# YuhuaXu/ImageMosaicing

Measured on AMD Instinct MI355X. Metric: image-pairs/sec (detect+match+H+warp), 4000x3000 UAV frames, higher is better.
Workload: dtype i16 fixed-point pyramid filtered in f32 (as the reference's OpenCV), f32 (RANSAC / warp coordinates), int8 MFMA with int32 accumulation (descriptor distances, exact), u8 (pixels); 1 GPU; C3: ONE 500-frame 4000x3000 UAV survey, pair window 2 (499 pairs), SIFT(2000,3,0.01,20) + exact BF match + 3x3 grid select + Ransac2D + MosaicImagesRefined warp; frames=500, pairs=499, frames_per_gpu=500, pairs_per_gpu=499

## Files before the change

imagemosaicing_amd/csrc/sift.hip:

```cpp
#include "common.h"
#include <memory>
#include "detmath.h"
#include <cmath>
#include <type_traits>

namespace {

constexpr int N_LAYERS = 3, N_LEVELS = 6, IMG_BORDER = 5, MAX_INTERP = 5, ORI_BINS = 36, MAX_OCT = 16;
constexpr int FIXPT_SCALE = 48;
constexpr float DOG_THRESHOLD_P1 = 21.0f;
constexpr float HIST_Q = 1024.0f;
constexpr int MAX_R = 16;
constexpr int SIFT_BATCH_MAX = MI355_SIFT_BATCH_MAX;
typedef int16_t lvl_t;

__host__ __device__ __forceinline__ int reflect101(int p, int n) {
    if (n == 1) return 0;
    while (p < 0 || p >= n) { if (p < 0) p = -p; else p = 2 * n - 2 - p; }
    return p;
}

typedef float v2f __attribute__((ext_vector_type(2)));
struct __attribute__((aligned(4))) uint2_a4 { unsigned x, y; };
typedef float v4f __attribute__((ext_vector_type(4)));
// ... 321 lines not shown
        }
    }
    __syncthreads();
    for (int item = tid; item < EH * (EW / 4); item += 256) {
        const int ly = item / (EW / 4), xg = item - ly * (EW / 4);
        const int r = y0 + ly;
        float cm[5][6], cn[5][6], mid[5][6], top[5][6], bot[5][6];
#pragma unroll
        for (int pl = 0; pl < 5; pl++) {
            const float* base = reinterpret_cast<const float*>(s_d4[pl]) + (ly + 1) * PC + 4 * xg + 4;
#pragma unroll
            for (int rr = -1; rr <= 1; rr++) {
                const float* q = base + rr * PC;
                const v4f c4 = *reinterpret_cast<const v4f*>(q);
                float v[6] = {q[-1], c4.x, c4.y, c4.z, c4.w, q[4]};
#pragma unroll
                for (int j = 0; j < 6; j++) { if (rr == -1) top[pl][j] = v[j]; else if (rr == 0) mid[pl][j] = v[j]; else bot[pl][j] = v[j]; }
            }
#pragma unroll
            for (int j = 0; j < 6; j++) {
                cm[pl][j] = fmaxf(fmaxf(top[pl][j], mid[pl][j]), bot[pl][j]);
                cn[pl][j] = fminf(fminf(top[pl][j], mid[pl][j]), bot[pl][j]);
            }
        }
        unsigned hit = 0;
#pragma unroll
        for (int k = 0; k < 4; k++) {
            const int j = k + 1;
#pragma unroll
            for (int layer = 1; layer <= N_LAYERS; layer++) {
                const float val = mid[layer][j];
                float mx = fmaxf(fmaxf(cm[layer - 1][j - 1], cm[layer - 1][j]), cm[layer - 1][j + 1]);
                mx = fmaxf(mx, fmaxf(fmaxf(cm[layer + 1][j - 1], cm[layer + 1][j]), cm[layer + 1][j + 1]));
                mx = fmaxf(mx, fmaxf(fmaxf(cm[layer][j - 1], cm[layer][j + 1]), fmaxf(top[layer][j], bot[layer][j])));
                float mn = fminf(fminf(cn[layer - 1][j - 1], cn[layer - 1][j]), cn[layer - 1][j + 1]);
                mn = fminf(mn, fminf(fminf(cn[layer + 1][j - 1], cn[layer + 1][j]), cn[layer + 1][j + 1]));
                mn = fminf(mn, fminf(fminf(cn[layer][j - 1], cn[layer][j + 1]), fminf(top[layer][j], bot[layer][j])));
                const float q = val > 0.0f ? mx : -mn;
                hit |= fabsf(val) >= fmaxf(q, DOG_THRESHOLD_P1) ? (1u << ((layer - 1) * 4 + k)) : 0u;
            }
        }
        unsigned cmask = 0;
#pragma unroll
        for (int k = 0; k < 4; k++) { const int c = x0 + 4 * xg + k; cmask |= (c >= IMG_BORDER && c < oc.w - IMG_BORDER) ? (0x111u << k) : 0u; }
        hit = (r >= IMG_BORDER && r < oc.h - IMG_BORDER) ? (hit & cmask) : 0u;
        while (hit) {
            const int bb = __builtin_ctz(hit); hit &= hit - 1;
            const int layer = bb / 4 + 1, c = x0 + 4 * xg + (bb & 3);
            const unsigned long long rec = ((unsigned long long)octave << 48) | ((unsigned long long)layer << 40) | ((unsigned long long)r << 20) | (unsigned long long)c;
            const unsigned slot = atomicAdd(&s_n, 1u);
            if (slot < ECAP) s_list[slot] = rec;
            else {
                const unsigned reg = ((unsigned)tile >> REG_SHIFT) & (NREG - 1);
                const unsigned g = atomicAdd(&count[reg * REG_STRIDE], 1u);
                if (g < cap) cand[(size_t)reg * cap + g] = rec; else *overflow = 1;
            }
        }
    }
    __syncthreads();
    const unsigned nloc = s_n < ECAP ? s_n : ECAP;
    const unsigned reg = ((unsigned)tile >> REG_SHIFT) & (NREG - 1);
    if (tid == 0 && nloc) s_base = atomicAdd(&count[reg * REG_STRIDE], nloc);
    __syncthreads();
    for (unsigned i = tid; i < nloc; i += 256) {
        const unsigned g = s_base + i;
        if (g < cap) cand[(size_t)reg * cap + g] = s_list[i] | (g < cube_cap ? (1ull << 63) : 0ull); else *overflow = 1;
    }
    for (unsigned idx = tid; idx < nloc * 27; idx += 256) {
        const unsigned ci = idx / 27, e = idx - ci * 27;
        const unsigned g = s_base + ci;
        if (g >= cube_cap) continue;
        const unsigned long long rec = s_list[ci];
        const int L0 = (int)((rec >> 40) & 0xff), R0 = (int)((rec >> 20) & 0xfffff), C0 = (int)(rec & 0xfffff);
        const int dl = (int)(e / 9) - 1, dr = (int)((e / 3) % 3) - 1, dc = (int)(e % 3) - 1;
        cube[((size_t)reg * 32 + e) * cube_cap + g] = reinterpret_cast<const float*>(s_d4[L0 + dl])[(R0 + dr - y0 + 1) * PC + (C0 + dc - x0) + 4];
    }
}

constexpr int XCAP = 512;
#ifndef MI355_XD
#define MI355_XD 2
#endif
constexpr int XD = MI355_XD;
#ifndef MI355_XWAVES
#define MI355_XWAVES 3
#endif
constexpr int XWAVES = MI355_XWAVES;
constexpr int XSW = 248;
typedef short s2 __attribute__((ext_vector_type(2)));
struct XRow { uint2 m[N_LEVELS]; };
struct XDog { s2 m[5][2]; };
__device__ __forceinline__ s2 as_s2(unsigned v) { return __builtin_bit_cast(s2, v); }
__device__ __forceinline__ unsigned as_u(s2 v) { return __builtin_bit_cast(unsigned, v); }
__device__ __forceinline__ s2 pmax(s2 a, s2 b) { return __builtin_elementwise_max(a, b); }
__device__ __forceinline__ s2 pmin(s2 a, s2 b) { return __builtin_elementwise_min(a, b); }
__device__ __forceinline__ unsigned dpp_lower(unsigned v) { return (unsigned)__builtin_amdgcn_update_dpp(0, (int)v, 0x138 , 0xf, 0xf, true); }
__device__ __forceinline__ unsigned dpp_upper(unsigned v) { return (unsigned)__builtin_amdgcn_update_dpp(0, (int)v, 0x130 , 0xf, 0xf, true); }

__device__ __forceinline__ unsigned xtest_row(const XDog& A, const XDog& B, const XDog& C, int xm, int clo, int chi, bool row_ok) {
    s2 hx[5][2], hn[5][2];
#pragma unroll
    for (int p = 0; p < 5; p++) {
        auto h3 = [](s2 c01, s2 c23, bool mx, s2& o01, s2& o23) {
            const unsigned u01 = as_u(c01), u23 = as_u(c23);
            const unsigned l23 = dpp_lower(u23), r01 = dpp_upper(u01);
            const s2 s_m0 = as_s2(__builtin_amdgcn_alignbit(u01, l23, 16));
            const s2 s_12 = as_s2(__builtin_amdgcn_alignbit(u23, u01, 16));
            const s2 s_34 = as_s2(__builtin_amdgcn_alignbit(r01, u23, 16));
            if (mx) { o01 = pmax(pmax(s_m0, c01), s_12); o23 = pmax(pmax(s_12, c23), s_34); }
            else    { o01 = pmin(pmin(s_m0, c01), s_12); o23 = pmin(pmin(s_12, c23), s_34); }
        };
        h3(pmax(pmax(A.m[p][0], B.m[p][0]), C.m[p][0]), pmax(pmax(A.m[p][1], B.m[p][1]), C.m[p][1]), true, hx[p][0], hx[p][1]);
        h3(pmin(pmin(A.m[p][0], B.m[p][0]), C.m[p][0]), pmin(pmin(A.m[p][1], B.m[p][1]), C.m[p][1]), false, hn[p][0], hn[p][1]);
    }
    unsigned hit = 0;
    const s2 t21 = {21, 21}, tm21 = {-21, -21};
#pragma unroll
    for (int layer = 1; layer <= N_LAYERS; layer++) {
#pragma unroll
        for (int r = 0; r < 2; r++) {
            const s2 val = B.m[layer][r];
            const s2 mx = pmax(pmax(pmax(hx[layer - 1][r], hx[layer][r]), hx[layer + 1][r]), t21);
            const s2 mn = pmin(pmin(pmin(hn[layer - 1][r], hn[layer][r]), hn[layer + 1][r]), tm21);
            const bool h0 = (val.x == mx.x) | (val.x == mn.x), h1 = (val.y == mx.y) | (val.y == mn.y);
            hit = (hit << 2) | (h0 ? 2u : 0u) | (h1 ? 1u : 0u);
        }
    }
    if (!row_ok || hit == 0) return 0u;
    unsigned out = 0;
#pragma unroll
    for (int b = 0; b < 12; b++) out |= ((hit >> (11 - b)) & 1u) << b;
    unsigned cmask = 0;
#pragma unroll
    for (int k = 0; k < 4; k++) cmask |= (xm + k >= clo && xm + k < chi) ? (0x111u << k) : 0u;
    return out & cmask;
}

struct XH { s2 hx[5][2], hn[5][2]; };
struct XCen { s2 v[3][2]; };
__device__ __forceinline__ void xrow_extremes(const XDog& d, XH& h, XCen& c) {
#pragma unroll
    for (int p = 0; p < 5; p++) {
        const unsigned u01 = as_u(d.m[p][0]), u23 = as_u(d.m[p][1]);
        const unsigned l23 = dpp_lower(u23), r01 = dpp_upper(u01);
        const s2 s_m0 = as_s2(__builtin_amdgcn_alignbit(u01, l23, 16));
        const s2 s_12 = as_s2(__builtin_amdgcn_alignbit(u23, u01, 16));
        const s2 s_34 = as_s2(__builtin_amdgcn_alignbit(r01, u23, 16));
        h.hx[p][0] = pmax(pmax(s_m0, d.m[p][0]), s_12); h.hx[p][1] = pmax(pmax(s_12, d.m[p][1]), s_34);
        h.hn[p][0] = pmin(pmin(s_m0, d.m[p][0]), s_12); h.hn[p][1] = pmin(pmin(s_12, d.m[p][1]), s_34);
    }
#pragma unroll
    for (int l = 0; l < 3; l++) { c.v[l][0] = d.m[l + 1][0]; c.v[l][1] = d.m[l + 1][1]; }
}
__device__ __forceinline__ unsigned xtest_rows(const XH& A, const XH& B, const XH& C, const XCen& cen, int xm, int clo, int chi, bool row_ok) {
    s2 hx[5][2], hn[5][2];
#pragma unroll
    for (int p = 0; p < 5; p++)
#pragma unroll
        for (int r = 0; r < 2; r++) { hx[p][r] = pmax(pmax(A.hx[p][r], B.hx[p][r]), C.hx[p][r]); hn[p][r] = pmin(pmin(A.hn[p][r], B.hn[p][r]), C.hn[p][r]); }
    unsigned hit = 0;
    const s2 t21 = {21, 21}, tm21 = {-21, -21};
#pragma unroll
    for (int layer = 1; layer <= N_LAYERS; layer++) {
#pragma unroll
        for (int r = 0; r < 2; r++) {
            const s2 val = cen.v[layer - 1][r];
            const s2 mx = pmax(pmax(pmax(hx[layer - 1][r], hx[layer][r]), hx[layer + 1][r]), t21);
            const s2 mn = pmin(pmin(pmin(hn[layer - 1][r], hn[layer][r]), hn[layer + 1][r]), tm21);
            const bool h0 = (val.x == mx.x) | (val.x == mn.x), h1 = (val.y == mx.y) | (val.y == mn.y);
            hit = (hit << 2) | (h0 ? 2u : 0u) | (h1 ? 1u : 0u);
        }
    }
    if (!row_ok || hit == 0) return 0u;
    unsigned out = 0;
#pragma unroll
    for (int b = 0; b < 12; b++) out |= ((hit >> (11 - b)) & 1u) << b;
    unsigned cmask = 0;
#pragma unroll
    for (int k = 0; k < 4; k++) cmask |= (xm + k >= clo && xm + k < chi) ? (0x111u << k) : 0u;
    return out & cmask;
}

__global__ __launch_bounds__(256) __attribute__((amdgpu_waves_per_eu(XWAVES, XWAVES)))
void extrema_stream(OctaveDev oc, int octave, unsigned long long* cand, unsigned* count, unsigned cap, unsigned* overflow, BatchStride bs,
                    float* cube, unsigned cube_cap, int L, int nstrip, int nseg, int nb, int xsw ) {
    const int lane = threadIdx.x & 63, wave = threadIdx.x >> 6;
    int unit = __builtin_amdgcn_readfirstlane(xcd_remap(blockIdx.x, gridDim.x) * 4 + wave);
    const int per = nstrip * nseg, fr = unit / per;
    if (fr >= nb) return;
    unit -= fr * per;
    {
        const size_t f = (size_t)fr;
#pragma unroll
        for (int l = 0; l < N_LEVELS; l++) oc.lv[l] += f * bs.pyr;
        cand += f * bs.cand; count += f * CCNT_STRIDE; overflow += f * CNT_STRIDE; cube += f * bs.cube;
    }
    const int seg = unit / nstrip, strip = unit - seg * nstrip;
    const int xs = strip * xsw, y0 = seg * L;
    const int lact = (oc.h - y0 < L) ? oc.h - y0 : L;
    const unsigned reg = (unsigned)unit & (NREG - 1);
    const int xm = xs - 4 + 4 * lane;
    const int xl = xm < 0 ? 0 : (xm < oc.w - 4 ? xm : oc.w - 4);
    int clo = xs > IMG_BORDER ? xs : IMG_BORDER, chi = xs + xsw < oc.w - IMG_BORDER ? xs + xsw : oc.w - IMG_BORDER;
    if (lane == 0 || lane == 63) { clo = 0; chi = 0; }
    const int hm1 = oc.h - 1;
    auto load_row = [&](int r, XRow& q) {
        r = r < 0 ? 0 : (r > hm1 ? hm1 : r);
        const size_t o = (size_t)r * oc.w + xl;
#pragma unroll
        for (int l = 0; l < N_LEVELS; l++) q.m[l] = *reinterpret_cast<const uint2*>(oc.lv[l] + o);
    };
    auto to_dog = [&](const XRow& q, XDog& d) {
#pragma unroll
        for (int p = 0; p < 5; p++) { d.m[p][0] = as_s2(q.m[p + 1].x) - as_s2(q.m[p].x); d.m[p][1] = as_s2(q.m[p + 1].y) - as_s2(q.m[p].y); }
    };
    __shared__ unsigned long long s_rec[4][XCAP];
    int nq = 0;
    auto wave_sync = [&]() { __builtin_amdgcn_fence(__ATOMIC_ACQ_REL, "wavefront"); __builtin_amdgcn_wave_barrier(); };
    auto flush = [&]() {
        if (nq == 0) return;
        wave_sync();
        unsigned base = 0;
        if (lane == 0) base = atomicAdd(&count[reg * REG_STRIDE], (unsigned)nq);
        base = __shfl(base, 0);
        for (int idx = lane; idx < nq; idx += 64) {
            const unsigned g = base + (unsigned)idx;
            if (g >= cap) { *overflow = 1; continue; }
            cand[(size_t)reg * cap + g] = s_rec[wave][idx];
        }
        wave_sync();
        nq = 0;
    };
    auto emit = [&](unsigned hit, int rc, auto in_loop) -> bool {
        constexpr bool IN_LOOP = decltype(in_loop)::value;
        const int nq0 = nq;
        while (__builtin_amdgcn_ballot_w64(hit != 0)) {
            const bool mine = hit != 0;
            const int bb = mine ? __builtin_ctz(hit) : 0;
            hit &= hit - 1;
            const unsigned long long m = __builtin_amdgcn_ballot_w64(mine);
            const int add = __builtin_popcountll(m);
            if (nq + add > XCAP) {
                if constexpr (IN_LOOP) { nq = nq0; return false; }
                else flush();
            }
            if (mine) {
                const int layer = bb / 4 + 1, c = xm + (bb & 3);
                s_rec[wave][nq + __builtin_popcountll(m & ((1ull << lane) - 1ull))] =
                    ((unsigned long long)octave << 48) | ((unsigned long long)layer << 40) | ((unsigned long long)rc << 20) | (unsigned long long)c;
            }
            nq += add;
        }
        return true;
    };
    XH win[3];
    XCen cen[3];
    XRow nxt[XD];
    {
        XRow q; XDog dq;
        load_row(y0 - 1, q); to_dog(q, dq); xrow_extremes(dq, win[0], cen[0]);
        load_row(y0, q); to_dog(q, dq); xrow_extremes(dq, win[1], cen[1]);
#pragma unroll
        for (int d = 0; d < XD; d++) load_row(y0 + 1 + d, nxt[d]);
    }
    int tb = 0, t_slow = -1;
    for (bool done = false; !done;) {
        for (;;) {
            if (tb >= lact) { done = true; break; }
            if (nq > XCAP / 2) break;
            auto step = [&](auto jc) -> bool {
                constexpr int j = decltype(jc)::value;
                const int tt = tb + j;
                if (tt >= lact) return false;
                const int rc = y0 + tt;
                XH& A = win[j % 3]; XH& B = win[(j + 1) % 3]; XH& Cc = win[(j + 2) % 3];
                { XDog dq; to_dog(nxt[j % XD], dq); xrow_extremes(dq, Cc, cen[(j + 2) % 3]); }
                load_row(rc + 1 + XD, nxt[j % XD]);
                const unsigned hit = xtest_rows(A, B, Cc, cen[(j + 1) % 3], xm, clo, chi, rc >= IMG_BORDER && rc < oc.h - IMG_BORDER);
                if (!emit(hit, rc, std::true_type{})) { t_slow = tt; return false; }
                return true;
            };
            if (!static_rows<0, 3 * XD>(step)) { done = true; break; }
            tb += 3 * XD;
        }
        flush();
    }
    if (t_slow >= 0) {
        for (int tt = t_slow; tt < lact; tt++) {
            const int rc = y0 + tt;
            XRow q; XDog A, B, Cc;
            load_row(rc - 1, q); to_dog(q, A);
            load_row(rc, q); to_dog(q, B);
            load_row(rc + 1, q); to_dog(q, Cc);
            emit(xtest_row(A, B, Cc, xm, clo, chi, rc >= IMG_BORDER && rc < oc.h - IMG_BORDER), rc, std::false_type{});
        }
        flush();
    }
}

__global__ __launch_bounds__(256) void refine_kernel(PyrDev P, const unsigned long long* cand_all, const unsigned* cand_counts, unsigned cand_cap, unsigned* cand_total,
                                                     float contrast_thr, float edge_thr, float sigma,
                                                     Refined* out, unsigned* out_count, unsigned out_cap, unsigned* out_resp, BatchStride bs,
                                                     const float* cube_all, unsigned cube_cap) {
    const size_t fr = blockIdx.z, foff = fr * bs.pyr;
    cube_all += fr * bs.cube;
    cand_all += fr * bs.cand; cand_counts += fr * CCNT_STRIDE; cand_total += fr * CNT_STRIDE;
    out += fr * bs.refined; out_count += fr * CNT_STRIDE; out_resp += fr * bs.refined;
    const unsigned reg = blockIdx.y;
    unsigned n = cand_counts[reg * REG_STRIDE];
    if (n > cand_cap) n = cand_cap;
    const unsigned long long* cand = cand_all + (size_t)reg * cand_cap;
    if (blockIdx.x == 0 && blockIdx.y == 0 && threadIdx.x < 64) {
        unsigned tot = cand_counts[threadIdx.x * REG_STRIDE];
        for (int off = 32; off > 0; off >>= 1) tot += __shfl_xor(tot, off);
        if (threadIdx.x == 0) cand_total[0] = tot;
    }
    for (unsigned i = blockIdx.x * blockDim.x + threadIdx.x; i < n; i += gridDim.x * blockDim.x) {
        const unsigned long long pk = cand[i];
        const int o = (int)((pk >> 48) & 0xff);
        int L = (int)((pk >> 40) & 0xff), R = (int)((pk >> 20) & 0xfffff), C = (int)(pk & 0xfffff);
        const unsigned start = ((unsigned)L << 28) | ((unsigned)R << 14) | (unsigned)C;
        const OctaveDev& oc = P.oc[o];
        auto dv = [&](int l, int r, int c) { return dogv(oc, foff, l, r, c); };
        FitOff f = {0.0f, 0.0f, 0.0f};
        int it = 0;
        bool alive = true, accepted = false;
        float contr = 0.0f;
        const bool from_cube = (pk >> 63) != 0;
        const bool can_gather = (oc.w & 1) == 0 && (foff & 1) == 0;
        float cv[27];
        auto gather = [&](int l, int r, int c) {
            const int a0 = (c - 1) & ~1, sh = ((c - 1) & 1) * 16;
            int v[4][9];
#pragma unroll
            for (int q = 0; q < 4; q++) {
                const lvl_t* lp = oc.lv[l - 1 + q] + foff;
#pragma unroll
                for (int dr = 0; dr < 3; dr++) {
                    const uint2_a4 wv = *reinterpret_cast<const uint2_a4*>(lp + (size_t)(r - 1 + dr) * oc.w + a0);
                    const unsigned long long ww = (((unsigned long long)wv.y << 32) | wv.x) >> sh;
                    v[q][dr * 3 + 0] = (int)(short)(ww & 0xffffu); v[q][dr * 3 + 1] = (int)(short)((ww >> 16) & 0xffffu); v[q][dr * 3 + 2] = (int)(short)((ww >> 32) & 0xffffu);
                }
            }
#pragma unroll
            for (int dl = 0; dl < 3; dl++)
#pragma unroll
                for (int e = 0; e < 9; e++) cv[dl * 9 + e] = (float)(v[dl + 1][e] - v[dl][e]);
        };
        if (from_cube || can_gather) {
            for (; it < MAX_INTERP; it++) {
                if (it == 0 && from_cube) {
                    const float* cb = cube_all + (size_t)reg * 32 * cube_cap + i;
#pragma unroll
                    for (int e = 0; e < 27; e++) cv[e] = cb[(size_t)e * cube_cap];
                } else if (can_gather) gather(L, R, C);
                else break;
                const int L0 = L, R0 = R, C0 = C;
                auto dvc = [&](int l, int r, int c) { return cv[(l - L0 + 1) * 9 + (r - R0 + 1) * 3 + (c - C0 + 1)]; };
                f = fit_step(dvc, L, R, C);
                const int stt = fit_state(f);
                if (stt == 1) { alive = false; break; }
                if (stt == 0) { accepted = fit_accept(dvc, L, R, C, f, contrast_thr, edge_thr, contr); alive = accepted; break; }
                C += (int)rintf(f.xc); R += (int)rintf(f.xr); L += (int)rintf(f.xi);
                if (L < 1 || L > N_LAYERS || C < IMG_BORDER || C >= oc.w - IMG_BORDER || R < IMG_BORDER || R >= oc.h - IMG_BORDER) { alive = false; break; }
            }
            if (!alive || (can_gather && !accepted)) continue;
        }
        if (!accepted) {
            for (; it < MAX_INTERP; it++) {
                f = fit_step(dv, L, R, C);
                const int stt = fit_state(f);
                if (stt == 0) break;
                if (stt == 1) { alive = false; break; }
                C += (int)rintf(f.xc); R += (int)rintf(f.xr); L += (int)rintf(f.xi);
                if (L < 1 || L > N_LAYERS || C < IMG_BORDER || C >= oc.w - IMG_BORDER || R < IMG_BORDER || R >= oc.h - IMG_BORDER) { alive = false; break; }
            }
            if (!alive || it >= MAX_INTERP) continue;
            if (!fit_accept(dv, L, R, C, f, contrast_thr, edge_thr, contr)) continue;
        }
        const size_t bit = ((size_t)R * oc.w + C) * 4 + (size_t)L;
        const unsigned mask = 1u << (bit & 31);
        if (!P.mins[o]) {
            const unsigned old = atomicOr(&P.claimed[o][fr * bs.claimed + (bit >> 5)], mask);
            if (old & mask) continue;
        }
        const unsigned long long act = __ballot(1);
        const int leader = __builtin_ctzll(act), lane_id = (int)(threadIdx.x & 63);
        unsigned slot = 0;
        if (lane_id == leader) slot = atomicAdd(out_count, (unsigned)__builtin_popcountll(act));
        slot = __shfl(slot, leader) + (unsigned)__builtin_popcountll(act & ((1ull << lane_id) - 1ull));
        if (slot < out_cap) {
            Refined rr;
            rr.o = o; rr.layer = L; rr.r = R; rr.c = C; rr.xi = f.xi; rr.xr = f.xr; rr.xc = f.xc; rr.contr = contr;
            rr.scl = sigma * det_exp2f(((float)L + f.xi) / (float)N_LAYERS);
            rr.start = start;
            out[slot] = rr;
            out_resp[slot] = __float_as_uint(fabsf(contr));
            if (P.mins[o]) atomicMin(&P.mins[o][fr * bs.mins + bit], start);
        } else if (!P.mins[o]) atomicAnd(&P.claimed[o][fr * bs.claimed + (bit >> 5)], ~mask);
    }
}

__device__ __forceinline__ void unclaim_body(const PyrDev& P, const Refined* ref, const unsigned* ref_count, unsigned ref_cap, const BatchStride& bs, size_t fr, unsigned first, unsigned step) {
    ref += fr * bs.refined; ref_count += fr * CNT_STRIDE;
    unsigned n = *ref_count;
    if (n > ref_cap) n = ref_cap;
    for (unsigned i = first; i < n; i += step) {
        const Refined rr = ref[i];
        const size_t bit = ((size_t)rr.r * P.oc[rr.o].w + rr.c) * 4 + (size_t)rr.layer;
        atomicAnd(&P.claimed[rr.o][fr * bs.claimed + (bit >> 5)], ~(1u << (bit & 31)));
    }
}

__global__ __launch_bounds__(256) void keepall_live_kernel(PyrDev P, const Refined* ref, const unsigned* ref_count, unsigned ref_cap, unsigned* ctrl, unsigned* list, BatchStride bs) {
    const size_t fr = blockIdx.y;
    ref += fr * bs.refined; ref_count += fr * CNT_STRIDE; ctrl += fr * CNT_STRIDE; list += fr * bs.refined;
    unsigned n = *ref_count;
    if (n > ref_cap) n = ref_cap;
    const int lane = threadIdx.x & 63;
    for (unsigned i0 = blockIdx.x * blockDim.x; i0 < n; i0 += gridDim.x * blockDim.x) {
        const unsigned i = i0 + threadIdx.x;
        bool take = false;
        if (i < n) {
            const Refined rr = ref[i];
            const size_t bit = ((size_t)rr.r * P.oc[rr.o].w + rr.c) * 4 + (size_t)rr.layer;
            take = P.mins[rr.o][fr * bs.mins + bit] == rr.start;
        }
        const unsigned long long m = __builtin_amdgcn_ballot_w64(take);
        if (m) {
            const int first = __builtin_ctzll(m);
            unsigned base = 0;
            if (lane == first) base = atomicAdd(&ctrl[2], (unsigned)__builtin_popcountll(m));
            base = __shfl(base, first);
            if (take) list[base + (unsigned)__builtin_popcountll(m & ((1ull << lane) - 1ull))] = i;
        }
    }
// ... 816 lines not shown
    MI_HIP(s->kresp.reserve(B * s->bs.kps * sizeof(unsigned)));
    MI_HIP(s->sel.reserve(B * s->bs.sel * sizeof(SelRec)));
    if (keepall) { MI_HIP(s->mins.reserve(B * ml * sizeof(unsigned))); MI_HIP(hipMemsetAsync(s->mins.p, 0xff, B * ml * sizeof(unsigned), s->stream)); }
    else s->mins.release();
    if (keepall) MI_HIP(s->ksort.reserve(B * s->ksort_stride * sizeof(unsigned long long)));
    else s->ksort.release();
    MI_HIP(s->counters.reserve(B * CNT_STRIDE * sizeof(unsigned)));
    MI_HIP(s->rhist.reserve(B * s->bs.refined * sizeof(unsigned)));
    MI_HIP(s->olist.reserve(B * s->bs.refined * sizeof(unsigned)));
    MI_HIP(s->ccnt.reserve(B * CCNT_STRIDE * sizeof(unsigned)));
    MI_HIP(s->cube.reserve(B * s->bs.cube * sizeof(float)));
    memset(&s->P, 0, sizeof(s->P));
    size_t fo = 0, co = 0, mo = 0;
    for (int o = 0; o < no; o++) {
        const int ow = w >> o, oh = h >> o;
        s->P.oc[o].w = ow; s->P.oc[o].h = oh;
        for (int i = 0; i < N_LEVELS; i++) { s->P.oc[o].lv[i] = s->pyr.as<lvl_t>() + fo; fo += up64((size_t)ow * oh); }
        s->P.claimed[o] = s->claimed.as<unsigned>() + co;
        co += (((size_t)ow * oh * 4 + 31) / 32 + 63) & ~(size_t)63;
        s->P.mins[o] = keepall ? s->mins.as<unsigned>() + mo : nullptr;
        mo += (size_t)ow * oh * 4;
    }
    s->P.n_oct = no; s->n_oct = no;
    s->w = w; s->h = h; s->nb = nb; s->keepall = keepall; s->kmax = kmax;
    return MI355_OK;
}


int mi_sift_extract_dev(mi355_ctx* ctx, int img_id, const uint8_t* d_bgr, int w, int h, int ws, int* n_kp) {
    if (ctx->p.n_octave_layers != N_LAYERS || ctx->p.sigma != 1.6f) { ctx->set_error("sift: this build implements nOctaveLayers=3, sigma=1.6 (the reference's SIFT(2000,3,0.01,20))"); return MI355_ERR_ARG; }
    if (ctx->p.nfeatures > 2048) { ctx->set_error("sift: nfeatures must be in [1,2048], or <= 0 for cv::SIFT's keep-all (up to keepall_max=" + std::to_string(ctx->keepall_max) + " keypoints per frame)"); return MI355_ERR_ARG; }
    const bool keepall = ctx->p.nfeatures <= 0;
    const int kmax = keepall ? ctx->keepall_max : 0;
    if (keepall && (w > 16384 || h > 16384)) { ctx->set_error("sift: keep-all frames are at most 16384 x 16384"); return MI355_ERR_ARG; }
    if ((size_t)w >= (1u << 20) || (size_t)h >= (1u << 20)) { ctx->set_error("sift: image too large"); return MI355_ERR_ARG; }
    if (w < 16 || h < 16) { ctx->set_error("sift: image too small"); return MI355_ERR_ARG; }
    if (ctx->sift_slots.empty()) {
        ctx->sift_slots.resize(SIFT_SLOTS_MAX, nullptr);
        MI_HIP(hipEventCreateWithFlags(&ctx->sift_in_ev, hipEventDisableTiming));
    }
    if (ctx->sift_next >= SIFT_SLOTS) ctx->sift_next = 0;
    const int slot = ctx->sift_next;
    if (!ctx->sift_slots[slot]) {
        ctx->sift_slots[slot] = new SiftWork();
        MI_HIP(hipStreamCreateWithFlags(&ctx->sift_slots[slot]->stream, hipStreamNonBlocking));
        MI_HIP(hipEventCreateWithFlags(&ctx->sift_slots[slot]->done, hipEventDisableTiming));
    }
    SiftWork* s = ctx->sift_slots[slot];
    int rc = MI355_OK;
    int nb = ctx->sift_batch < 1 ? 1 : (ctx->sift_batch > SIFT_BATCH_MAX ? SIFT_BATCH_MAX : ctx->sift_batch);
    {
        static size_t total_mem = [] { size_t fr = 0, tot = 0; return hipMemGetInfo(&fr, &tot) == hipSuccess ? tot : (size_t)0; }();
        const double per_frame = 60.0 * (double)w * (double)h;
        if (total_mem) {
            const int fit = (int)(0.6 * (double)total_mem / ((keepall ? 1.4 : 1.0) * per_frame) / (double)SIFT_SLOTS);
            if (fit < nb) nb = fit < 1 ? 1 : fit;
        }
        if (keepall && nb > 8) nb = 8;
    }
    if (!s->pend.empty() && (s->w != w || s->h != h || s->nb != nb || s->keepall != keepall || s->kmax != kmax)) { rc = sift_run_batch(ctx, s); if (rc != MI355_OK) return rc; }
    rc = sift_prepare(ctx, s, w, h, nb, keepall, kmax);
    if (rc != MI355_OK) return rc;
    auto fit = ctx->feats.find(img_id);
    if (fit != ctx->feats.end() && fit->second.pending) { rc = mi_resolve_features(ctx); if (rc != MI355_OK) return rc; }
    Features& f = ctx->feats[img_id];
    f.w = w; f.h = h;
    MI_HIP(f.kp.reserve(sizeof(mi355_keypoint) * (size_t)(keepall ? kmax : 2048)));
    MI_HIP(f.d8.reserve((size_t)128 * (size_t)(keepall ? kmax : 2048)));
    f.pending = true; f.h_cnt = nullptr; f.ready = nullptr; f.n = 0;
    s->pend.push_back({img_id, d_bgr, ws, ctx->pend_event});
    if ((int)s->pend.size() >= nb) {
        rc = sift_run_batch(ctx, s);
        if (rc != MI355_OK) return rc;
    }
    if (ctx->pinned_used >= PINNED_CHUNK * 64) {
        rc = mi_resolve_features(ctx);
        if (rc != MI355_OK) return rc;
        ctx->pinned_used = 0;
    }
    if (n_kp) {
        rc = mi_resolve_features(ctx);
        if (rc != MI355_OK) return rc;
        *n_kp = f.n;
    }
    return MI355_OK;
}

static int sift_run_batch(mi355_ctx* ctx, SiftWork* s) {
    std::vector<SiftWork::Pend> pend;
    pend.swap(s->pend);
    const int n = (int)pend.size();
    if (n == 0) return MI355_OK;
    ctx->sift_next = (ctx->sift_next + 1) % SIFT_SLOTS;
    const hipStream_t st = s->stream;
    const hipStream_t tt = st;
    const int w = s->w, h = s->h;
    const int nf = ctx->p.nfeatures;
    const BatchStride bs = s->bs;
    MI_HIP(hipEventRecord(ctx->sift_in_ev, ctx->stream));
    MI_HIP(hipStreamWaitEvent(st, ctx->sift_in_ev, 0));
    const bool serial_heavy = ctx->serial_heavy != 0;
    if (serial_heavy && ctx->heavy_ev_valid) MI_HIP(hipStreamWaitEvent(st, ctx->heavy_ev, 0));
    unsigned* cnt = s->counters.as<unsigned>();
    MI_HIP(hipMemsetAsync(cnt, 0, (size_t)n * CNT_STRIDE * sizeof(unsigned), st));
    MI_HIP(hipMemsetAsync(s->ccnt.p, 0, (size_t)n * CCNT_STRIDE * sizeof(unsigned), st));
    FrameOuts outs;
    memset(&outs, 0, sizeof(outs));
    std::vector<Features*> fs(n);
    for (int k = 0; k < n; k++) {
        fs[k] = &ctx->feats[pend[k].img_id];
        outs.kp[k] = fs[k]->kp.as<mi355_keypoint>(); outs.d8[k] = fs[k]->d8.as<uint8_t>();
    }
    auto blur_args = [&](const OctaveDev& oc) {
        Blur16Args a; memset(&a, 0, sizeof(a));
        a.w = oc.w; a.h = oc.h; a.tiles_x = (oc.w + T16W - 1) / T16W; a.tiles_y = (oc.h + T16H - 1) / T16H;
        a.fstride = bs.pyr; a.nb = n;
        return a;
    };
    bool ds_fused = false;
    for (int o = 0; o < s->n_oct; o++) {
        const OctaveDev& oc = s->P.oc[o];
        const double level_bytes = (double)oc.w * oc.h * sizeof(lvl_t) * n;
        if (o == 0) {
            Blur16Args a = blur_args(oc);
            for (int k = 0; k < n; k++) { a.bgr[k] = pend[k].d_bgr; a.bgr_ws[k] = pend[k].ws; }
            a.dst = oc.lv[0];
            memcpy(a.k, s->kern0, sizeof(float) * (2 * s->radius0 + 1));
            const bool streams = blur_streams(a, true, s->radius0, ctx->blur_stream);
            ProfScope ps(ctx, streams ? "gauss_stream" : "gauss", level_bytes + (double)w * h * 3.0 * n, st);
            if (!launch_blur<true>(st, s->radius0, a, ctx->blur_stream)) { ctx->set_error("sift: unsupported kernel radius"); return MI355_ERR_FAILED; }
        } else if (!ds_fused) {
            const OctaveDev& pv = s->P.oc[o - 1];
            ProfScope ps(ctx, "downsample", level_bytes * 2.0, st);
            hipLaunchKernelGGL(downsample16, dim3((oc.w + 63) / 64, (oc.h + 3) / 4, n), dim3(256), 0, st, pv.lv[N_LAYERS], pv.w, oc.lv[0], oc.w, oc.h, bs.pyr);
        }
        ds_fused = false;
        for (int i = 1; i < N_LEVELS; i++) {
            Blur16Args a = blur_args(oc);
            a.src = oc.lv[i - 1]; a.dst = oc.lv[i];
            memcpy(a.k, s->kern[i], sizeof(float) * (2 * s->radius[i] + 1));
            if (i == N_LAYERS && o + 1 < s->n_oct && (oc.w & 3) == 0 && (s->P.oc[o + 1].w == (oc.w >> 1)) && (s->P.oc[o + 1].h == (oc.h >> 1))) {
                a.ds = s->P.oc[o + 1].lv[0]; ds_fused = true;
                if (!blur_streams(a, false, s->radius[i], ctx->blur_stream)) {
                    Blur16Args b = a; b.ds = nullptr;
                    if (blur_streams(b, false, s->radius[i], ctx->blur_stream)) { a.ds = nullptr; ds_fused = false; }
                }
            }
            const bool streams = blur_streams(a, false, s->radius[i], ctx->blur_stream);
            ProfScope ps(ctx, streams ? "gauss_stream" : "gauss", level_bytes * 2.0, st);
            if (!launch_blur<false>(st, s->radius[i], a, ctx->blur_stream)) { ctx->set_error("sift: unsupported kernel radius"); return MI355_ERR_FAILED; }
        }
        {
            ProfScope ps(ctx, "extrema", level_bytes * 6.0, st);
            const bool xs = ctx->blur_stream && (oc.w & 3) == 0 && oc.w >= ctx->xstream_min_w && oc.h >= ctx->xstream_min_w * 3 / 4 && n >= ctx->xstream_min_frames;
            if (xs) {
                const int nstrip = (oc.w + XSW - 1) / XSW;
                const int xsw = ((oc.w + nstrip - 1) / nstrip + 3) & ~3;
                int nseg = 1, L = oc.h;
                for (int k = 2; k >= 1; k--) {
                    const int ns = (1024 * XWAVES * k) / (nstrip * n);
                    if (ns < 1) continue;
                    const int l = (oc.h + ns - 1) / ns;
                    if (l >= 64 || k == 1) { L = l < 64 ? 64 : l; break; }
                }
                nseg = (oc.h + L - 1) / L;
                hipLaunchKernelGGL(extrema_stream, dim3((nstrip * nseg * n + 3) / 4), dim3(256), 0, st,
                                   oc, o, s->cand.as<unsigned long long>(), s->ccnt.as<unsigned>(), s->cand_cap, cnt + 4, bs, s->cube.as<float>(), s->cube_cap, L, nstrip, nseg, n, xsw);
            } else {
                hipLaunchKernelGGL(extrema_kernel, dim3(((oc.w + EW - 1) / EW) * ((oc.h + EH - 1) / EH), n), dim3(256), 0, st,
                                   oc, o, s->cand.as<unsigned long long>(), s->ccnt.as<unsigned>(), s->cand_cap, cnt + 4, bs, s->cube.as<float>(), s->cube_cap);
            }
        }
    }
    if (serial_heavy) {
        if (!ctx->heavy_ev) MI_HIP(hipEventCreateWithFlags(&ctx->heavy_ev, hipEventDisableTiming));
        MI_HIP(hipEventRecord(ctx->heavy_ev, st)); ctx->heavy_ev_valid = true;
    }
    {
        ProfScope ps(ctx, "refine", 0.0, tt);
        static const int refine_gx = [] { const char* e = getenv("MI355_REFINE_GX"); return e ? atoi(e) : 2; }();
        hipLaunchKernelGGL(refine_kernel, dim3(refine_gx, NREG, n), dim3(256), 0, tt, s->P, s->cand.as<unsigned long long>(), s->ccnt.as<unsigned>(), s->cand_cap, cnt + 0,
                           ctx->p.contrast_threshold, ctx->p.edge_threshold, 1.6f, s->refined.as<Refined>(), cnt + 1, s->ref_cap, s->rhist.as<unsigned>(), bs, s->cube.as<float>(), s->cube_cap);
    }
    if (s->keepall) {
        {
            ProfScope ps(ctx, "kp_select", 0.0, tt);
            hipLaunchKernelGGL(keepall_live_kernel, dim3(256, n), dim3(256), 0, tt, s->P, s->refined.as<Refined>(), cnt + 1, s->ref_cap, cnt + 8, s->olist.as<unsigned>(), bs);
            hipLaunchKernelGGL(keepall_reset_kernel, dim3(256, n), dim3(256), 0, tt, s->P, s->refined.as<Refined>(), cnt + 1, s->ref_cap, bs);
        }
        {
            ProfScope ps(ctx, "orient", 0.0, tt);
            hipLaunchKernelGGL(orient_kernel, dim3(ctx->num_cu * 4, n), dim3(256), 0, tt, s->P, s->refined.as<Refined>(), cnt + 1, s->ref_cap,
                               s->kps.as<KpRec>(), s->kresp.as<unsigned>(), cnt + 2, s->kp_cap, cnt + 8, 0, bs, s->olist.as<unsigned>());
        }
        {
            ProfScope ps(ctx, "topk", 0.0, tt);
            const unsigned kmax = (unsigned)s->kmax;
            if (ctx->keepall_order == 1) {
                hipLaunchKernelGGL(keepall_output_kernel, dim3((kmax + 255) / 256, n), dim3(256), 0, tt, s->kps.as<KpRec>(), cnt + 2, s->kp_cap, kmax, outs, s->sel.as<SelRec>(),
                                   reinterpret_cast<int*>(cnt + 3), reinterpret_cast<int*>(cnt + 4), bs);
            } else {
                hipLaunchKernelGGL(keepall_sort_tiles_kernel, dim3((kmax + KA_TILE - 1) / KA_TILE, n), dim3(1024), 0, tt, s->kps.as<KpRec>(), cnt + 2, s->kp_cap, kmax,
                                   s->ksort.as<unsigned long long>(), s->ksort_stride, outs, s->sel.as<SelRec>(), bs);
                hipLaunchKernelGGL(keepall_place_kernel, dim3((kmax + 255) / 256, n), dim3(256), 0, tt, s->kps.as<KpRec>(), cnt + 2, s->kp_cap, kmax,
                                   s->ksort.as<const unsigned long long>(), s->ksort_stride, outs, s->sel.as<SelRec>(), reinterpret_cast<int*>(cnt + 3), reinterpret_cast<int*>(cnt + 4), bs);
            }
        }
    } else {
    {
        ProfScope ps(ctx, "kp_select", 0.0, tt);
        hipLaunchKernelGGL(select_unclaim_kernel, dim3(1 + UNCLAIM_WGS, n), dim3(1024), 0, tt, s->P, s->refined.as<Refined>(), bs, s->rhist.as<unsigned>(), cnt + 1, s->ref_cap, (unsigned)nf + 256u, cnt + 8,
                           bs.refined, s->olist.as<unsigned>());
    }
    for (int pass = 0; pass < 2; pass++) {
        {
            ProfScope ps(ctx, "orient", 0.0, tt);
            hipLaunchKernelGGL(orient_kernel, dim3(ctx->num_cu * 4, n), dim3(256), 0, tt, s->P, s->refined.as<Refined>(), cnt + 1, s->ref_cap,
                               s->kps.as<KpRec>(), s->kresp.as<unsigned>(), cnt + 2, s->kp_cap, cnt + 8, pass, bs, s->olist.as<unsigned>());
        }
        {
            ProfScope ps(ctx, "topk", 0.0, tt);
            hipLaunchKernelGGL(topk_kernel, dim3(n), dim3(1024), 0, tt, s->kps.as<KpRec>(), s->kresp.as<unsigned>(), cnt + 2, s->kp_cap, nf,
                               outs, s->sel.as<SelRec>(), reinterpret_cast<int*>(cnt + 3), reinterpret_cast<int*>(cnt + 4), cnt + 8, pass, bs);
        }
    }
    }
    {
        ProfScope ps(ctx, "describe", 0.0, tt);
        hipLaunchKernelGGL(describe_kernel, dim3(((int)bs.sel + 3) / 4, n), dim3(256), 0, tt, s->P, s->sel.as<SelRec>(), reinterpret_cast<const int*>(cnt + 3), outs, bs);
    }
    MI_HIP(hipGetLastError());
    { int rc = mi_finish_features_batch(ctx, fs.data(), n, reinterpret_cast<const int*>(cnt + 3), (int)CNT_STRIDE, tt, s->keepall ? s->kmax : 2048); if (rc != MI355_OK) return rc; }
    {
        if (ctx->pinned_used % PINNED_CHUNK + (size_t)n > PINNED_CHUNK) ctx->pinned_used += PINNED_CHUNK - ctx->pinned_used % PINNED_CHUNK;
        int* h0 = nullptr;
        for (int k = 0; k < n; k++) {
            int* hc = pinned_slot(ctx);
            if (!hc) { ctx->set_error("sift: pinned alloc failed"); return MI355_ERR_NOMEM; }
            if (k == 0) h0 = hc;
            Features& f = *fs[k];
            f.h_cnt = hc; f.pending = true; f.n = 0;
            f.caps[0] = 0xffffffffu; f.caps[1] = s->ref_cap; f.caps[2] = s->kp_cap;
            f.kp_limit = s->keepall ? s->kmax : 0;
        }
        MI_HIP(hipMemcpy2DAsync(h0, 8 * sizeof(int), cnt, CNT_STRIDE * sizeof(unsigned), 8 * sizeof(unsigned), (size_t)n, hipMemcpyDeviceToHost, tt));
    }
    MI_HIP(hipEventRecord(s->done, tt));
    {
        if (ctx->batch_events_used >= ctx->batch_events.size()) {
            hipEvent_t e = nullptr;
            MI_HIP(hipEventCreateWithFlags(&e, hipEventDisableTiming));
            ctx->batch_events.push_back(e);
        }
        hipEvent_t e = ctx->batch_events[ctx->batch_events_used++];
        MI_HIP(hipEventRecord(e, tt));
        for (int k = 0; k < n; k++) fs[k]->ready = e;
    }
    for (int k = 0; k < n; k++) if (pend[k].ev) MI_HIP(hipEventRecord(pend[k].ev, tt));
    return MI355_OK;
}

int mi_sift_flush_if_parked(mi355_ctx* ctx, hipEvent_t ev) {
    for (SiftWork* s : ctx->sift_slots) {
        if (!s) continue;
        for (const SiftWork::Pend& p : s->pend) if (p.ev == ev) return sift_run_batch(ctx, s);
    }
    return MI355_OK;
}
```

Before: 3905 image-pairs/s.

## Share vertical max/min across row pairs and use buffer loads in extrema stream

Reworks the streaming DoG extrema test so that the elementwise max/min of the two middle rows is computed once and reused by two consecutive output rows, instead of reducing all three rows for every row. It also shares the cross-layer max/min between adjacent layers, writes hit bits directly in output order so the bit-reversal loop goes away, and folds the threshold clamp into the pair reduction. Row loads switch from 64-bit flat pointer arithmetic to buffer loads with 32-bit offsets, and the unroll length is doubled when XD is odd so the row-pair rotation lines up. A size guard keeps the streaming path off for levels of 2 GiB or more, and an ISA counting script is added to scratch.

```diff
diff --git a/imagemosaicing_amd/csrc/sift.hip b/imagemosaicing_amd/csrc/sift.hip
--- a/imagemosaicing_amd/csrc/sift.hip
+++ b/imagemosaicing_amd/csrc/sift.hip
@@ -497,33 +497,41 @@
 #pragma unroll
     for (int l = 0; l < 3; l++) { c.v[l][0] = d.m[l + 1][0]; c.v[l][1] = d.m[l + 1][1]; }
 }
-__device__ __forceinline__ unsigned xtest_rows(const XH& A, const XH& B, const XH& C, const XCen& cen, int xm, int clo, int chi, bool row_ok) {
+__device__ __forceinline__ void xpair_rows(XH& y, const XH& n) {
+    const s2 t21 = {21, 21}, tm21 = {-21, -21};
+#pragma unroll
+    for (int p = 0; p < 5; p++)
+#pragma unroll
+        for (int r = 0; r < 2; r++) {
+            y.hx[p][r] = pmax(y.hx[p][r], n.hx[p][r]); y.hn[p][r] = pmin(y.hn[p][r], n.hn[p][r]);
+            if (p == 2) { y.hx[p][r] = pmax(y.hx[p][r], t21); y.hn[p][r] = pmin(y.hn[p][r], tm21); }
+        }
+}
+__device__ __forceinline__ unsigned xtest_rows(const XH& P, const XH& R, const XCen& cen, int xm, int clo, int chi, bool row_ok) {
     s2 hx[5][2], hn[5][2];
 #pragma unroll
     for (int p = 0; p < 5; p++)
 #pragma unroll
-        for (int r = 0; r < 2; r++) { hx[p][r] = pmax(pmax(A.hx[p][r], B.hx[p][r]), C.hx[p][r]); hn[p][r] = pmin(pmin(A.hn[p][r], B.hn[p][r]), C.hn[p][r]); }
+        for (int r = 0; r < 2; r++) { hx[p][r] = pmax(P.hx[p][r], R.hx[p][r]); hn[p][r] = pmin(P.hn[p][r], R.hn[p][r]); }
     unsigned hit = 0;
-    const s2 t21 = {21, 21}, tm21 = {-21, -21};
-#pragma unroll
-    for (int layer = 1; layer <= N_LAYERS; layer++) {
-#pragma unroll
-        for (int r = 0; r < 2; r++) {
-            const s2 val = cen.v[layer - 1][r];
-            const s2 mx = pmax(pmax(pmax(hx[layer - 1][r], hx[layer][r]), hx[layer + 1][r]), t21);
-            const s2 mn = pmin(pmin(pmin(hn[layer - 1][r], hn[layer][r]), hn[layer + 1][r]), tm21);
-            const bool h0 = (val.x == mx.x) | (val.x == mn.x), h1 = (val.y == mx.y) | (val.y == mn.y);
-            hit = (hit << 2) | (h0 ? 2u : 0u) | (h1 ? 1u : 0u);
+#pragma unroll
+    for (int r = 0; r < 2; r++) {
+        const s2 x12 = pmax(hx[1][r], hx[2][r]), x23 = pmax(hx[2][r], hx[3][r]);
+        const s2 n12 = pmin(hn[1][r], hn[2][r]), n23 = pmin(hn[2][r], hn[3][r]);
+        const s2 mx[3] = {pmax(hx[0][r], x12), pmax(x12, hx[3][r]), pmax(x23, hx[4][r])};
+        const s2 mn[3] = {pmin(hn[0][r], n12), pmin(n12, hn[3][r]), pmin(n23, hn[4][r])};
+#pragma unroll
+        for (int l = 0; l < 3; l++) {
+            const s2 val = cen.v[l][r];
+            const bool h0 = (val.x == mx[l].x) | (val.x == mn[l].x), h1 = (val.y == mx[l].y) | (val.y == mn[l].y);
+            hit |= (h0 ? 1u : 0u) << (4 * l + 2 * r) | (h1 ? 1u : 0u) << (4 * l + 2 * r + 1);
         }
     }
     if (!row_ok || hit == 0) return 0u;
-    unsigned out = 0;
-#pragma unroll
-    for (int b = 0; b < 12; b++) out |= ((hit >> (11 - b)) & 1u) << b;
     unsigned cmask = 0;
 #pragma unroll
     for (int k = 0; k < 4; k++) cmask |= (xm + k >= clo && xm + k < chi) ? (0x111u << k) : 0u;
-    return out & cmask;
+    return hit & cmask;
 }
 
 __global__ __launch_bounds__(256) __attribute__((amdgpu_waves_per_eu(XWAVES, XWAVES)))
@@ -549,11 +557,16 @@
     int clo = xs > IMG_BORDER ? xs : IMG_BORDER, chi = xs + xsw < oc.w - IMG_BORDER ? xs + xsw : oc.w - IMG_BORDER;
     if (lane == 0 || lane == 63) { clo = 0; chi = 0; }
     const int hm1 = oc.h - 1;
+    typedef unsigned u2v __attribute__((ext_vector_type(2)));
+    __amdgpu_buffer_rsrc_t lvr[N_LEVELS];
+#pragma unroll
+    for (int l = 0; l < N_LEVELS; l++) lvr[l] = __builtin_amdgcn_make_buffer_rsrc(oc.lv[l], 0, oc.w * oc.h * (int)sizeof(lvl_t), 0x00020000 );
+    const unsigned xoff = (unsigned)xl * (unsigned)sizeof(lvl_t), pitch = (unsigned)oc.w * (unsigned)sizeof(lvl_t);
     auto load_row = [&](int r, XRow& q) {
         r = r < 0 ? 0 : (r > hm1 ? hm1 : r);
-        const size_t o = (size_t)r * oc.w + xl;
-#pragma unroll
-        for (int l = 0; l < N_LEVELS; l++) q.m[l] = *reinterpret_cast<const uint2*>(oc.lv[l] + o);
+        const unsigned o = (unsigned)r * pitch;
+#pragma unroll
+        for (int l = 0; l < N_LEVELS; l++) { const u2v v = __builtin_amdgcn_raw_buffer_load_b64(lvr[l], xoff, o, 0); q.m[l] = make_uint2(v.x, v.y); }
     };
     auto to_dog = [&](const XRow& q, XDog& d) {
 #pragma unroll
@@ -598,6 +611,7 @@
         }
         return true;
     };
+    constexpr int XU = (XD % 2 == 0 ? 3 : 6) * XD;
     XH win[3];
     XCen cen[3];
     XRow nxt[XD];
@@ -618,15 +632,17 @@
                 const int tt = tb + j;
                 if (tt >= lact) return false;
                 const int rc = y0 + tt;
-                XH& A = win[j % 3]; XH& B = win[(j + 1) % 3]; XH& Cc = win[(j + 2) % 3];
-                { XDog dq; to_dog(nxt[j % XD], dq); xrow_extremes(dq, Cc, cen[(j + 2) % 3]); }
+                constexpr int sx = (3 - (j % 6) / 2) % 3;
+                XH& X = win[sx]; XH& Y = win[(sx + 1) % 3]; XH& N = win[(sx + 2) % 3];
+                { XDog dq; to_dog(nxt[j % XD], dq); xrow_extremes(dq, j % 2 == 0 ? N : X, cen[(j + 2) % 3]); }
                 load_row(rc + 1 + XD, nxt[j % XD]);
-                const unsigned hit = xtest_rows(A, B, Cc, cen[(j + 1) % 3], xm, clo, chi, rc >= IMG_BORDER && rc < oc.h - IMG_BORDER);
+                if (j % 2 == 0) xpair_rows(Y, N);
+                const unsigned hit = xtest_rows(Y, X, cen[(j + 1) % 3], xm, clo, chi, rc >= IMG_BORDER && rc < oc.h - IMG_BORDER);
                 if (!emit(hit, rc, std::true_type{})) { t_slow = tt; return false; }
                 return true;
             };
-            if (!static_rows<0, 3 * XD>(step)) { done = true; break; }
-            tb += 3 * XD;
+            if (!static_rows<0, XU>(step)) { done = true; break; }
+            tb += XU;
         }
         flush();
     }
@@ -1749,7 +1765,7 @@
         }
         {
             ProfScope ps(ctx, "extrema", level_bytes * 6.0, st);
-            const bool xs = ctx->blur_stream && (oc.w & 3) == 0 && oc.w >= ctx->xstream_min_w && oc.h >= ctx->xstream_min_w * 3 / 4 && n >= ctx->xstream_min_frames;
+            const bool xs = ctx->blur_stream && (oc.w & 3) == 0 && (size_t)oc.w * oc.h * sizeof(lvl_t) < (1ull << 31) && oc.w >= ctx->xstream_min_w && oc.h >= ctx->xstream_min_w * 3 / 4 && n >= ctx->xstream_min_frames;
             if (xs) {
                 const int nstrip = (oc.w + XSW - 1) / XSW;
                 const int xsw = ((oc.w + nstrip - 1) / nstrip + 3) & ~3;
diff --git a/scratch/xstream_isa_count.py b/scratch/xstream_isa_count.py
--- /dev/null
+++ b/scratch/xstream_isa_count.py
@@ -0,0 +1,31 @@
+import re
+import sys
+
+s = open(sys.argv[1]).read()
+m = re.search(r'^(_ZN\S*extrema_stream\S*):.*?^\.Lfunc_end\d+:', s, re.S | re.M)
+lines = m.group(0).split('\n')
+
+
+def label(j):
+    for i, l in enumerate(lines):
+        if re.search(r'integral_constantIiLi%dEEEEbS\d_\.exit' % j, l) and l.lstrip().startswith((';', '.LBB')):
+            return i
+    return None
+
+
+for j in (1, 2, 3):
+    a, b = label(j - 1), label(j)
+    if a is None or b is None or b < a:
+        print('step', j, ': not contiguous in this listing'); continue
+    body = [l.split()[0] for l in lines[a:b] if l.startswith('\t') and not l.startswith('\t.')]
+    v = [x for x in body if x.startswith('v_')]
+    cls = {'dog': 0, 'shuffle': 0, 'pk_maxmin': 0, 'cmp': 0, 'addr64': 0, 'other': 0}
+    for x in v:
+        if x == 'v_pk_sub_i16': cls['dog'] += 1
+        elif x in ('v_mov_b32_dpp', 'v_alignbit_b32'): cls['shuffle'] += 1
+        elif x in ('v_pk_max_i16', 'v_pk_min_i16'): cls['pk_maxmin'] += 1
+        elif x.startswith('v_cmp_eq_u16'): cls['cmp'] += 1
+        elif x == 'v_lshl_add_u64': cls['addr64'] += 1
+        else: cls['other'] += 1
+    print('step', j, 'valu', len(v), cls, '| salu', len([x for x in body if x.startswith('s_') and x not in ('s_waitcnt', 's_nop')]),
+          'loads', len([x for x in body if x.startswith(('global_load', 'buffer_load'))]))
```

Result: no change. 3890 image-pairs/s (-0.4%).
